# JDAI-CV/CoTNet

Measured on AMD Instinct MI355X. Metric: images/sec CoTNet-50 224^2 fwd+bwd, higher is better.
Workload: dtype bf16; 1 GPU; cotnet50 224x224 fwd+bwd+SGD-nesterov, random init, 1000 classes, NCHW synthetic ImageNet-shaped input resident in HBM; per_gpu_batch=80, global_batch=80, parallelism=dp1, layout=nchw, precision=bf16 weights+activations, fp32 master weights / norm params, fused flat SGD, conv1x1=hip, conv3x3=hip, group_norm9=hip, cot_layer_single_node_enabled=True, grad_sync=none (1 GPU)

## Files before the change

### cotnet_amd/csrc/stem7x7.hip

```cpp
#include "cot_common.h"
#include "mfma_common.h"
#include "cot_host.h"

namespace cot {

constexpr int kStemK = 147, kStemKp = 160, kStemCo = 64;

__device__ __forceinline__ void stem_tap(int k, int& ci, int& kh, int& kw) {
    ci = k / 49;
    const int r = k - 49 * ci;
    kh = r / 7;
    kw = r - 7 * kh;
}

__global__ void __launch_bounds__(256)
stem7x7_fwd_mfma(const bf16_t* __restrict__ x, const bf16_t* __restrict__ w, bf16_t* __restrict__ y, int H, int W, int Ho,
                 int Wo, int tiles_per_image, int64_t total_waves) {
    extern __shared__ __attribute__((aligned(16))) char cot_smem[];
    bf16_t* As = reinterpret_cast<bf16_t*>(cot_smem);
    for (int i = threadIdx.x; i < kStemCo * kStemKp; i += blockDim.x) {
        const int m = i / kStemKp, k = i - m * kStemKp;
        As[i] = k < kStemK ? w[m * kStemK + k] : (bf16_t)0.0f;
    }
    __syncthreads();
    const int64_t wid = (int64_t)blockIdx.x * 4 + (threadIdx.x >> 6);
    if (wid >= total_waves) return;
    const int lane = threadIdx.x & 63, j = lane & 15, g = lane >> 4;
    const int n = uniform((int)(wid / tiles_per_image)), tile = uniform((int)(wid % tiles_per_image));
    const int HWo = Ho * Wo;
    const int p0 = tile * 64 + 4 * j;
    const int oh = min(p0, HWo - 1) / Wo, ow0 = min(p0, HWo - 1) % Wo;
    const int ih0 = 2 * oh - 3, iw0 = 2 * ow0 - 3;
    const bf16_t* xn = x + (int64_t)n * 3 * H * W;

    f32x4_t acc[4][4];
#pragma unroll
    for (int a = 0; a < 4; ++a)
#pragma unroll
        for (int c = 0; c < 4; ++c) acc[a][c] = f32x4_t{0.f, 0.f, 0.f, 0.f};

#pragma unroll
    for (int step = 0; step < kStemKp / 32; ++step) {
        const int kb = 32 * step + 8 * g;
        bf16x8_t bfrag[4];
#pragma unroll
        for (int e = 0; e < 8; ++e) {
            const int k = kb + e;
            int ci, kh, kw;
            stem_tap(min(k, kStemK - 1), ci, kh, kw);
            const int ih = ih0 + kh;
            const bool rok = k < kStemK && ih >= 0 && ih < H && p0 < HWo;
            const bf16_t* row = xn + ((int64_t)ci * H + (rok ? ih : 0)) * W;
#pragma unroll
            for (int cs = 0; cs < 4; ++cs) {
                const int iw = iw0 + 2 * cs + kw;
                bfrag[cs][e] = (rok && iw >= 0 && iw < W) ? row[iw] : (bf16_t)0.0f;
            }
        }
#pragma unroll
        for (int a = 0; a < 4; ++a) {
            bf16x8_t af;
            __builtin_memcpy(&af, __builtin_assume_aligned(As + (16 * a + j) * kStemKp + kb, 16), 16);
#pragma unroll
            for (int cs = 0; cs < 4; ++cs) acc[a][cs] = COT_MFMA_16X16X32_BF16(af, bfrag[cs], acc[a][cs]);
        }
    }
    if (p0 >= HWo) return;
#pragma unroll
    for (int a = 0; a < 4; ++a)
#pragma unroll
        for (int i = 0; i < 4; ++i) {
            const int co = 16 * a + 4 * g + i;
            bf16_t o[4];
#pragma unroll
            for (int cs = 0; cs < 4; ++cs) o[cs] = (bf16_t)acc[a][cs][i];
            store_piece<4, 8>(y + ((int64_t)n * kStemCo + co) * HWo + p0, o, HWo - p0);
        }
}

__global__ void __launch_bounds__(256)
stem7x7_fwd_lds(const bf16_t* __restrict__ x, const bf16_t* __restrict__ w, bf16_t* __restrict__ y, int H, int W, int Ho, int Wo,
                int tiles_per_image, int NR, int RS) {
    constexpr int WS = 168;
    extern __shared__ __attribute__((aligned(16))) char cot_smem[];
    bf16_t* As = reinterpret_cast<bf16_t*>(cot_smem);
    uint16_t* toff = reinterpret_cast<uint16_t*>(As + kStemCo * WS);
    bf16_t* patch = reinterpret_cast<bf16_t*>(toff + kStemKp);
    const int tid = threadIdx.x, lane = tid & 63, wave = tid >> 6, j = lane & 15, g = lane >> 4;
    const int n = blockIdx.x / tiles_per_image, tile = blockIdx.x - n * tiles_per_image;
    const int HWo = Ho * Wo;
    const int pfirst = tile * 256;
    const int ih_base = 2 * (pfirst / Wo) - 3;
    for (int i = tid; i < kStemCo * WS; i += 256) {
        const int m = i / WS, k = i - m * WS;
        As[i] = k < kStemK ? w[m * kStemK + k] : (bf16_t)0.0f;
    }
    if (tid < kStemKp) {
        int ci, kh, kw;
        stem_tap(min(tid, kStemK - 1), ci, kh, kw);
        toff[tid] = (uint16_t)((ci * NR + kh) * RS + kw);
    }
    {
        const int cpr = RS / 8, chunks = 3 * NR * cpr;
        const bf16_t* xn = x + (int64_t)n * 3 * H * W;
        for (int q = tid; q < chunks; q += 256) {
            const int row = q / cpr, c = q - row * cpr;
            const int ci = row / NR, ih = ih_base + (row - ci * NR);
            Vec<bf16_t, 8> v;
#pragma unroll
            for (int e = 0; e < 8; ++e) v.v[e] = (bf16_t)0.0f;
            if (c >= 1 && 8 * (c - 1) < W && ih >= 0 && ih < H) v = ldv<bf16_t, 8>(xn + ((int64_t)ci * H + ih) * W + 8 * (c - 1));
            stv<bf16_t, 8>(patch + (int64_t)row * RS + 8 * c, v);
        }
    }
    __syncthreads();
    const int p0 = pfirst + wave * 64 + 4 * j;
    const int pc = min(p0, HWo - 4);
    const int oh = pc / Wo, ow0 = pc - oh * Wo;
    const uint16_t* pl = reinterpret_cast<const uint16_t*>(patch) + (2 * oh - 3 - ih_base) * RS + 8 + 2 * ow0 - 3;

    f32x4_t acc[4][4];
#pragma unroll
    for (int a = 0; a < 4; ++a)
#pragma unroll
        for (int c = 0; c < 4; ++c) acc[a][c] = f32x4_t{0.f, 0.f, 0.f, 0.f};
#pragma unroll
    for (int step = 0; step < kStemKp / 32; ++step) {
        const int kb = 32 * step + 8 * g;
        uint16_t to[8];
        __builtin_memcpy(to, __builtin_assume_aligned(toff + kb, 16), 16);
        uint16_t q[4][8];
#pragma unroll
        for (int e = 0; e < 8; ++e) {
            const uint16_t* pe = pl + to[e];
            const bool kok = step < 4 || kb + e < kStemK;
#pragma unroll
            for (int cs = 0; cs < 4; ++cs) {
                const uint16_t v = pe[2 * cs];
                q[cs][e] = kok ? v : (uint16_t)0;
            }
        }
        bf16x8_t bfrag[4];
#pragma unroll
        for (int cs = 0; cs < 4; ++cs) __builtin_memcpy(&bfrag[cs], q[cs], 16);
#pragma unroll
        for (int a = 0; a < 4; ++a) {
            bf16x8_t af;
            __builtin_memcpy(&af, __builtin_assume_aligned(As + (16 * a + j) * WS + kb, 16), 16);
#pragma unroll
            for (int cs = 0; cs < 4; ++cs) acc[a][cs] = COT_MFMA_16X16X32_BF16(af, bfrag[cs], acc[a][cs]);
        }
    }
    if (p0 >= HWo) return;
#pragma unroll
    for (int a = 0; a < 4; ++a)
#pragma unroll
        for (int i = 0; i < 4; ++i) {
            const int co = 16 * a + 4 * g + i;
            bf16_t o[4];
#pragma unroll
            for (int cs = 0; cs < 4; ++cs) o[cs] = (bf16_t)acc[a][cs][i];
            store_piece<4, 8>(y + ((int64_t)n * kStemCo + co) * HWo + p0, o, HWo - p0);
        }
}

__global__ void __launch_bounds__(256)
stem7x7_wgrad_mfma(const bf16_t* __restrict__ gy, const bf16_t* __restrict__ x, float* __restrict__ part, int N, int H,
                   int W, int Ho, int Wo, int S, int spi, int64_t total_waves) {
    const int64_t wid = (int64_t)blockIdx.x * 4 + (threadIdx.x >> 6);
    if (wid >= total_waves) return;
    const int lane = threadIdx.x & 63, i16 = lane & 15, lg = lane >> 4;
    const int cb = uniform((int)(wid & 1)), s = uniform((int)(wid >> 1));
    const int HWo = Ho * Wo;
    const int T = N * spi, t0 = (int)((int64_t)T * s / S), t1 = (int)((int64_t)T * (s + 1) / S);
    int tci[5], tkh[5], tkw[5];
    bool tok[5];
#pragma unroll
    for (int q = 0; q < 5; ++q) {
        const int k = cb * 80 + q * 16 + i16;
        tok[q] = k < kStemK;
        stem_tap(min(k, kStemK - 1), tci[q], tkh[q], tkw[q]);
    }
    f32x4_t acc[4][5];
#pragma unroll
    for (int a = 0; a < 4; ++a)
#pragma unroll
        for (int q = 0; q < 5; ++q) acc[a][q] = f32x4_t{0.f, 0.f, 0.f, 0.f};

    for (int t = t0; t < t1; ++t) {
        const int n = t / spi, st = t - n * spi;
        const int p = st * 32 + 8 * lg;
        const int oh = p / Wo, ow = p - oh * Wo;
        bf16x8_t af[4], bfr[5];
#pragma unroll
        for (int a = 0; a < 4; ++a)
            __builtin_memcpy(&af[a], __builtin_assume_aligned(gy + ((int64_t)n * kStemCo + 16 * a + i16) * HWo + p, 16), 16);
#pragma unroll
        for (int q = 0; q < 5; ++q) {
            const int ih = 2 * oh - 3 + tkh[q];
            const bool rok = tok[q] && ih >= 0 && ih < H;
            const bf16_t* row = x + (((int64_t)n * 3 + tci[q]) * H + (rok ? ih : 0)) * W;
            const int iw0 = 2 * ow - 3 + tkw[q];
#pragma unroll
            for (int e = 0; e < 8; ++e) {
                const int iw = iw0 + 2 * e;
                bfr[q][e] = (rok && iw >= 0 && iw < W) ? row[iw] : (bf16_t)0.0f;
            }
        }
#pragma unroll
        for (int a = 0; a < 4; ++a)
#pragma unroll
            for (int q = 0; q < 5; ++q) acc[a][q] = COT_MFMA_16X16X32_BF16(af[a], bfr[q], acc[a][q]);
    }
    float* ps = part + (int64_t)s * kStemCo * kStemK;
#pragma unroll
    for (int a = 0; a < 4; ++a)
#pragma unroll
        for (int i = 0; i < 4; ++i) {
            const int co = 16 * a + 4 * lg + i;
#pragma unroll
            for (int q = 0; q < 5; ++q) {
                const int k = cb * 80 + q * 16 + i16;
                if (k < kStemK) ps[co * kStemK + k] = acc[a][q][i];
            }
        }
}

__global__ void __launch_bounds__(256)
stem7x7_wgrad_lds(const bf16_t* __restrict__ gy, const bf16_t* __restrict__ x, float* __restrict__ part, int N, int H, int W, int Ho,
                  int Wo, int S, int RS) {
    extern __shared__ __attribute__((aligned(16))) char cot_smem[];
    bf16_t* const patch = reinterpret_cast<bf16_t*>(cot_smem);
    const int tid = threadIdx.x, lane = tid & 63, wave = tid >> 6, i16 = lane & 15, lg = lane >> 4;
    const int cb = wave & 1, mh = wave >> 1, s = blockIdx.x;
    const int HWo = Ho * Wo, ppi = Ho / 2;
    const int T = N * ppi, t0 = (int)((int64_t)T * s / S), t1 = (int)((int64_t)T * (s + 1) / S);
    const int cpr = RS / 8, chunks = 27 * cpr;
    constexpr int NCH = 4;
    int toff[5];
    bool tok[5];
#pragma unroll
    for (int q = 0; q < 5; ++q) {
        const int k = cb * 80 + q * 16 + i16;
        int ci, kh, kw;
        stem_tap(min(k, kStemK - 1), ci, kh, kw);
        tok[q] = k < kStemK;
        toff[q] = (ci * 9 + kh) * RS + 8 - 3 + kw;
    }
    f32x4_t acc[2][5];
#pragma unroll
    for (int a = 0; a < 2; ++a)
#pragma unroll
        for (int q = 0; q < 5; ++q) acc[a][q] = f32x4_t{0.f, 0.f, 0.f, 0.f};
    Vec<bf16_t, 8> hold[NCH];
    auto fetch = [&](int t) __attribute__((always_inline)) {
        const int n = t / ppi, pr = t - n * ppi, ih0 = 4 * pr - 3;
        const bf16_t* xn = x + (int64_t)n * 3 * H * W;
#pragma unroll
        for (int j = 0; j < NCH; ++j) {
            const int qd = j * 256 + tid;
#pragma unroll
            for (int e = 0; e < 8; ++e) hold[j].v[e] = (bf16_t)0.0f;
            if (qd < chunks) {
                const int row = qd / cpr, c = qd - row * cpr;
                const int ci = row / 9, ih = ih0 + (row - ci * 9);
                if (c >= 1 && 8 * (c - 1) < W && ih >= 0 && ih < H) hold[j] = ldv<bf16_t, 8>(xn + ((int64_t)ci * H + ih) * W + 8 * (c - 1));
            }
        }
    };
    auto put = [&](int buf) __attribute__((always_inline)) {
#pragma unroll
        for (int j = 0; j < NCH; ++j) {
            const int qd = j * 256 + tid;
            if (qd < chunks) stv<bf16_t, 8>(patch + (int64_t)buf * 27 * RS + (int64_t)qd * 8, hold[j]);
        }
    };
    if (t0 < t1) {
        fetch(t0);
        put(0);
    }
    __syncthreads();
    for (int t = t0; t < t1; ++t) {
        const int buf = (t - t0) & 1;
        if (t + 1 < t1) fetch(t + 1);
        const int n = t / ppi, pr = t - n * ppi;
        const uint16_t* pb = reinterpret_cast<const uint16_t*>(patch) + buf * 27 * RS;
        const bf16_t* gyn = gy + (int64_t)n * kStemCo * HWo + (int64_t)(2 * pr) * Wo;
        for (int ks = 0; ks < 2 * Wo; ks += 32) {
            const int p = ks + 8 * lg;
            const int r2 = p >= Wo ? 1 : 0, ow = p - r2 * Wo;
            const int pbase = 2 * r2 * RS + 2 * ow;
            bf16x8_t af[2], bfr[5];
#pragma unroll
            for (int a = 0; a < 2; ++a)
                __builtin_memcpy(&af[a], __builtin_assume_aligned(gyn + (int64_t)(32 * mh + 16 * a + i16) * HWo + p, 16), 16);
#pragma unroll
            for (int q = 0; q < 5; ++q) {
                const uint16_t* pe = pb + pbase + toff[q];
                uint16_t v[8];
#pragma unroll
                for (int e = 0; e < 8; ++e) v[e] = tok[q] ? pe[2 * e] : (uint16_t)0;
                __builtin_memcpy(&bfr[q], v, 16);
            }
#pragma unroll
            for (int a = 0; a < 2; ++a)
#pragma unroll
                for (int q = 0; q < 5; ++q) acc[a][q] = COT_MFMA_16X16X32_BF16(af[a], bfr[q], acc[a][q]);
        }
        if (t + 1 < t1) put(buf ^ 1);
        __syncthreads();
    }
    float* ps = part + (int64_t)s * kStemCo * kStemK;
#pragma unroll
    for (int a = 0; a < 2; ++a)
#pragma unroll
        for (int i = 0; i < 4; ++i) {
            const int co = 32 * mh + 16 * a + 4 * lg + i;
#pragma unroll
            for (int q = 0; q < 5; ++q) {
                const int k = cb * 80 + q * 16 + i16;
                if (k < kStemK) ps[co * kStemK + k] = acc[a][q][i];
            }
        }
}

static bool stem_geometry(int H, int W, int* Ho, int* Wo) {
    *Ho = (H + 6 - 7) / 2 + 1;
    *Wo = (W + 6 - 7) / 2 + 1;
    return H > 0 && W > 0 && (*Wo % 8) == 0 && ((*Ho * *Wo) % 32) == 0;
}

int g_stem_lds = 1;
static int stem_wgrad_lds_slices(int N, int H, int W, int Ho, int Wo) {
    if (!g_stem_lds || W % 8 != 0 || (2 * Wo) % 32 != 0 || (Ho & 1) || 27 * ((W + 16) / 8) > 4 * 256) return 0;
    const int64_t T = (int64_t)N * (Ho / 2);
    int64_t S = T / 8;
    if (S > 1024) S = 1024;
    return (int)(S < 1 ? 1 : S);
}
int stem7x7_splits(int N, int H, int W) {
    int Ho, Wo;
    if (!stem_geometry(H, W, &Ho, &Wo)) return 0;
    if (const int sl = stem_wgrad_lds_slices(N, H, W, Ho, Wo)) return sl;
    const int64_t T = (int64_t)N * (Ho * Wo / 32);
    int64_t S = 512;
    if (S > T / 16) S = T / 16;
    return (int)(S < 1 ? 1 : S);
}

int stem7x7_forward(const void* x, const void* w, void* y, int N, int H, int W, hipStream_t stream) {
    int Ho, Wo;
    if (!stem_geometry(H, W, &Ho, &Wo)) return COT_ERR_UNSUPPORTED;
    if (g_stem_lds && W % 8 == 0 && Wo % 4 == 0 && (Ho * Wo) % 4 == 0) {
        const int rows = 255 / Wo + 2, NR = 2 * (rows - 1) + 7, RS = W + 16;
        const size_t lds = ((size_t)kStemCo * 168 + kStemKp + (size_t)3 * NR * RS) * 2;
        if (lds <= 64 * 1024 && (3 * NR + 6) * RS + 8 < 65536) {
            const int tiles = ceil_div(Ho * Wo, 256);
            COT_LAUNCH(stem7x7_fwd_lds, dim3((unsigned)((int64_t)N * tiles)), dim3(256), lds, stream, (const bf16_t*)x, (const bf16_t*)w,
                       (bf16_t*)y, H, W, Ho, Wo, tiles, NR, RS);
            return check_launch("stem7x7_fwd_lds");
        }
    }
    const int tpi = ceil_div(Ho * Wo, 64);
    const int64_t waves = (int64_t)N * tpi;
    COT_LAUNCH(stem7x7_fwd_mfma, dim3((unsigned)ceil_div64(waves, 4)), dim3(256), kStemCo * kStemKp * 2, stream,
               (const bf16_t*)x, (const bf16_t*)w, (bf16_t*)y, H, W, Ho, Wo, tpi, waves);
    return check_launch("stem7x7_fwd_mfma");
}

int stem7x7_wgrad(const void* gy, const void* x, void* gw, float* workspace, int N, int H, int W, hipStream_t stream) {
    int Ho, Wo;
    if (!stem_geometry(H, W, &Ho, &Wo)) return COT_ERR_UNSUPPORTED;
    if (const int SL = stem_wgrad_lds_slices(N, H, W, Ho, Wo)) {
        const int RS = W + 16;
        COT_LAUNCH(stem7x7_wgrad_lds, dim3((unsigned)SL), dim3(256), (size_t)2 * 27 * RS * 2, stream, (const bf16_t*)gy, (const bf16_t*)x,
                   workspace, N, H, W, Ho, Wo, SL, RS);
        int rc = check_launch("stem7x7_wgrad_lds");
        if (rc) return rc;
        return conv1x1_wgrad_reduce_launch(workspace, SL, kStemCo, kStemK, 0, gw, nullptr, stream);
    }
    const int S = stem7x7_splits(N, H, W), spi = Ho * Wo / 32;
    const int64_t waves = (int64_t)S * 2;
    COT_LAUNCH(stem7x7_wgrad_mfma, dim3((unsigned)ceil_div64(waves, 4)), dim3(256), 0, stream, (const bf16_t*)gy,
               (const bf16_t*)x, workspace, N, H, W, Ho, Wo, S, spi, waves);
    int rc = check_launch("stem7x7_wgrad_mfma");
    if (rc) return rc;
    return conv1x1_wgrad_reduce_launch(workspace, S, kStemCo, kStemK, 0, gw, nullptr, stream);
}

}
```

Before: 5961 images/s.

## Restructure 7x7 stem conv around kernel-row K packing with persistent, prefetched tiles

Reorders the stem reduction dimension by kernel row: each 8-wide K chunk holds one (channel, kh) row of 7 taps plus a zero pad, so B fragments come from contiguous vector reads instead of per-element gathers. The weights are pre-swizzled into per-lane MFMA fragment order in LDS. The forward LDS kernel becomes persistent, processing 8 tiles per workgroup and prefetching the next tile's input patch into registers while the current tile computes. Weight-gradient patches are split into even/odd column planes and run through a ring-buffered gy load loop, and the slice cap drops from 1024 to 512. K grows from 160 to 192 slots, so more MFMA work is padding, and the forward kernel may request more than 64KB of LDS, which can lower occupancy.

```diff
diff --git a/cotnet_amd/csrc/stem7x7.hip b/cotnet_amd/csrc/stem7x7.hip
--- a/cotnet_amd/csrc/stem7x7.hip
+++ b/cotnet_amd/csrc/stem7x7.hip
@@ -1,10 +1,15 @@
 #include "cot_common.h"
 #include "mfma_common.h"
+#include "conv_lds_common.h"
 #include "cot_host.h"
 
 namespace cot {
 
 constexpr int kStemK = 147, kStemKp = 160, kStemCo = 64;
+constexpr int kStemRows = 21, kStemSteps = 6;
+constexpr int kStemWFrag = 4 * kStemSteps * 64;
+constexpr int kStemTilesPerWg = 8;
+constexpr int kStemWgradSlices = 512;
 
 __device__ __forceinline__ void stem_tap(int k, int& ci, int& kh, int& kw) {
     ci = k / 49;
@@ -13,15 +18,28 @@
     kw = r - 7 * kh;
 }
 
+__device__ __forceinline__ void stem_stage_weights(const bf16_t* __restrict__ w, bf16_t* Af, int tid) {
+    for (int f = tid; f < kStemWFrag; f += 256) {
+        const int q = f >> 6, lane = f & 63, a = q / kStemSteps, s = q - a * kStemSteps;
+        const int co = 16 * a + (lane & 15), r = 4 * s + (lane >> 4);
+        Vec<bf16_t, 8> v;
+#pragma unroll
+        for (int e = 0; e < 8; ++e) v.v[e] = (bf16_t)0.0f;
+        if (r < kStemRows) {
+            const Vec<bf16_t, 7> t = ldv<bf16_t, 7>(w + co * kStemK + 7 * r);
+#pragma unroll
+            for (int e = 0; e < 7; ++e) v.v[e] = t.v[e];
+        }
+        stv<bf16_t, 8>(Af + 8 * f, v);
+    }
+}
+
 __global__ void __launch_bounds__(256)
 stem7x7_fwd_mfma(const bf16_t* __restrict__ x, const bf16_t* __restrict__ w, bf16_t* __restrict__ y, int H, int W, int Ho,
                  int Wo, int tiles_per_image, int64_t total_waves) {
     extern __shared__ __attribute__((aligned(16))) char cot_smem[];
-    bf16_t* As = reinterpret_cast<bf16_t*>(cot_smem);
-    for (int i = threadIdx.x; i < kStemCo * kStemKp; i += blockDim.x) {
-        const int m = i / kStemKp, k = i - m * kStemKp;
-        As[i] = k < kStemK ? w[m * kStemK + k] : (bf16_t)0.0f;
-    }
+    bf16_t* Af = reinterpret_cast<bf16_t*>(cot_smem);
+    stem_stage_weights(w, Af, threadIdx.x);
     __syncthreads();
     const int64_t wid = (int64_t)blockIdx.x * 4 + (threadIdx.x >> 6);
     if (wid >= total_waves) return;
@@ -40,27 +58,25 @@
         for (int c = 0; c < 4; ++c) acc[a][c] = f32x4_t{0.f, 0.f, 0.f, 0.f};
 
 #pragma unroll
-    for (int step = 0; step < kStemKp / 32; ++step) {
-        const int kb = 32 * step + 8 * g;
+    for (int step = 0; step < kStemSteps; ++step) {
+        const int r = 4 * step + g, rc = min(r, kStemRows - 1);
+        const int ci = (rc >= 7) + (rc >= 14), ih = ih0 + rc - 7 * ci;
+        const bool rok = r < kStemRows && ih >= 0 && ih < H && p0 < HWo;
+        const bf16_t* row = xn + ((int64_t)ci * H + (rok ? ih : 0)) * W;
         bf16x8_t bfrag[4];
 #pragma unroll
-        for (int e = 0; e < 8; ++e) {
-            const int k = kb + e;
-            int ci, kh, kw;
-            stem_tap(min(k, kStemK - 1), ci, kh, kw);
-            const int ih = ih0 + kh;
-            const bool rok = k < kStemK && ih >= 0 && ih < H && p0 < HWo;
-            const bf16_t* row = xn + ((int64_t)ci * H + (rok ? ih : 0)) * W;
-#pragma unroll
-            for (int cs = 0; cs < 4; ++cs) {
-                const int iw = iw0 + 2 * cs + kw;
+        for (int cs = 0; cs < 4; ++cs) {
+#pragma unroll
+            for (int e = 0; e < 7; ++e) {
+                const int iw = iw0 + 2 * cs + e;
                 bfrag[cs][e] = (rok && iw >= 0 && iw < W) ? row[iw] : (bf16_t)0.0f;
             }
+            bfrag[cs][7] = (bf16_t)0.0f;
         }
 #pragma unroll
         for (int a = 0; a < 4; ++a) {
             bf16x8_t af;
-            __builtin_memcpy(&af, __builtin_assume_aligned(As + (16 * a + j) * kStemKp + kb, 16), 16);
+            __builtin_memcpy(&af, __builtin_assume_aligned(Af + 8 * ((a * kStemSteps + step) * 64 + lane), 16), 16);
 #pragma unroll
             for (int cs = 0; cs < 4; ++cs) acc[a][cs] = COT_MFMA_16X16X32_BF16(af, bfrag[cs], acc[a][cs]);
         }
@@ -78,90 +94,134 @@
         }
 }
 
+constexpr int kStemHold = 5;
+constexpr int kStemRing = 4;
 __global__ void __launch_bounds__(256)
 stem7x7_fwd_lds(const bf16_t* __restrict__ x, const bf16_t* __restrict__ w, bf16_t* __restrict__ y, int H, int W, int Ho, int Wo,
-                int tiles_per_image, int NR, int RS) {
-    constexpr int WS = 168;
+                int tiles_per_image, int NR, int RS, int64_t total_tiles, int tpw) {
     extern __shared__ __attribute__((aligned(16))) char cot_smem[];
-    bf16_t* As = reinterpret_cast<bf16_t*>(cot_smem);
-    uint16_t* toff = reinterpret_cast<uint16_t*>(As + kStemCo * WS);
-    bf16_t* patch = reinterpret_cast<bf16_t*>(toff + kStemKp);
+    bf16_t* Af = reinterpret_cast<bf16_t*>(cot_smem);
+    bf16_t* patch = Af + 8 * kStemWFrag;
     const int tid = threadIdx.x, lane = tid & 63, wave = tid >> 6, j = lane & 15, g = lane >> 4;
-    const int n = blockIdx.x / tiles_per_image, tile = blockIdx.x - n * tiles_per_image;
     const int HWo = Ho * Wo;
-    const int pfirst = tile * 256;
-    const int ih_base = 2 * (pfirst / Wo) - 3;
-    for (int i = tid; i < kStemCo * WS; i += 256) {
-        const int m = i / WS, k = i - m * WS;
-        As[i] = k < kStemK ? w[m * kStemK + k] : (bf16_t)0.0f;
-    }
-    if (tid < kStemKp) {
-        int ci, kh, kw;
-        stem_tap(min(tid, kStemK - 1), ci, kh, kw);
-        toff[tid] = (uint16_t)((ci * NR + kh) * RS + kw);
-    }
-    {
-        const int cpr = RS / 8, chunks = 3 * NR * cpr;
+    stem_stage_weights(w, Af, tid);
+    int roff[kStemSteps];
+#pragma unroll
+    for (int s = 0; s < kStemSteps; ++s) {
+        const int r = min(4 * s + g, kStemRows - 1), ci = (r >= 7) + (r >= 14);
+        roff[s] = ((ci * NR + r - 7 * ci) * RS) >> 1;
+    }
+    const int cpr = RS / 8, chunks = 3 * NR * cpr, drow = 256 / cpr, dcol = 256 - drow * cpr;
+    const int row_first = tid / cpr, col_first = tid - row_first * cpr;
+    auto next_piece = [&](int& row, int& c) __attribute__((always_inline)) {
+        row += drow;
+        c += dcol;
+        if (c >= cpr) {
+            c -= cpr;
+            ++row;
+        }
+    };
+    auto load_piece = [&](uint32_t (&v)[5], const bf16_t* xn, int ih_base, int row, int c) __attribute__((always_inline)) {
+        const int ci = (row >= NR) + (row >= 2 * NR), ih = ih_base + (row - ci * NR);
+#pragma unroll
+        for (int e = 0; e < 5; ++e) v[e] = 0u;
+        if (ih >= 0 && ih < H) {
+            const bf16_t* xr = xn + ((int64_t)ci * H + ih) * W + 8 * c;
+            if (c >= 2 && 8 * (c - 2) < W) __builtin_memcpy(&v[0], __builtin_assume_aligned(xr - 12, 8), 8);
+            if (c >= 1 && 8 * (c - 1) < W) __builtin_memcpy(&v[2], __builtin_assume_aligned(xr - 8, 16), 12);
+        }
+    };
+    auto make_piece = [&](uint32_t (&o)[4], const uint32_t (&v)[5]) __attribute__((always_inline)) {
+#pragma unroll
+        for (int e = 0; e < 4; ++e) o[e] = (v[e] >> 16) | (v[e + 1] << 16);
+    };
+    uint32_t hold[kStemHold][5];
+    auto fetch = [&](int64_t t) __attribute__((always_inline)) {
+        const int n = (int)(t / tiles_per_image), tile = (int)(t - (int64_t)n * tiles_per_image);
+        const int ih_base = 2 * (tile * 256 / Wo) - 3;
         const bf16_t* xn = x + (int64_t)n * 3 * H * W;
-        for (int q = tid; q < chunks; q += 256) {
-            const int row = q / cpr, c = q - row * cpr;
-            const int ci = row / NR, ih = ih_base + (row - ci * NR);
-            Vec<bf16_t, 8> v;
-#pragma unroll
-            for (int e = 0; e < 8; ++e) v.v[e] = (bf16_t)0.0f;
-            if (c >= 1 && 8 * (c - 1) < W && ih >= 0 && ih < H) v = ldv<bf16_t, 8>(xn + ((int64_t)ci * H + ih) * W + 8 * (c - 1));
-            stv<bf16_t, 8>(patch + (int64_t)row * RS + 8 * c, v);
-        }
-    }
-    __syncthreads();
-    const int p0 = pfirst + wave * 64 + 4 * j;
-    const int pc = min(p0, HWo - 4);
-    const int oh = pc / Wo, ow0 = pc - oh * Wo;
-    const uint16_t* pl = reinterpret_cast<const uint16_t*>(patch) + (2 * oh - 3 - ih_base) * RS + 8 + 2 * ow0 - 3;
-
-    f32x4_t acc[4][4];
-#pragma unroll
-    for (int a = 0; a < 4; ++a)
-#pragma unroll
-        for (int c = 0; c < 4; ++c) acc[a][c] = f32x4_t{0.f, 0.f, 0.f, 0.f};
-#pragma unroll
-    for (int step = 0; step < kStemKp / 32; ++step) {
-        const int kb = 32 * step + 8 * g;
-        uint16_t to[8];
-        __builtin_memcpy(to, __builtin_assume_aligned(toff + kb, 16), 16);
-        uint16_t q[4][8];
-#pragma unroll
-        for (int e = 0; e < 8; ++e) {
-            const uint16_t* pe = pl + to[e];
-            const bool kok = step < 4 || kb + e < kStemK;
+        int row = row_first, c = col_first;
+#pragma unroll
+        for (int i = 0; i < kStemHold; ++i) {
+            if (tid + 256 * i < chunks) load_piece(hold[i], xn, ih_base, row, c);
+            next_piece(row, c);
+        }
+    };
+    const int64_t t0 = (int64_t)blockIdx.x * tpw, t1 = t0 + tpw < total_tiles ? t0 + tpw : total_tiles;
+    if (t0 < t1) fetch(t0);
+    for (int64_t t = t0; t < t1; ++t) {
+        const int n = (int)(t / tiles_per_image), tile = (int)(t - (int64_t)n * tiles_per_image);
+        const int pfirst = tile * 256;
+        const int ih_base = 2 * (pfirst / Wo) - 3;
+        __syncthreads();
+        {
+            int row = row_first, c = col_first;
+#pragma unroll
+            for (int i = 0; i < kStemHold; ++i) {
+                if (tid + 256 * i < chunks) {
+                    uint32_t o[4];
+                    make_piece(o, hold[i]);
+                    __builtin_memcpy(__builtin_assume_aligned(patch + row * RS + 8 * c, 16), o, 16);
+                }
+                next_piece(row, c);
+            }
+            const bf16_t* xn = x + (int64_t)n * 3 * H * W;
+            for (int q = tid + 256 * kStemHold; q < chunks; q += 256) {
+                uint32_t v[5], o[4];
+                load_piece(v, xn, ih_base, row, c);
+                make_piece(o, v);
+                __builtin_memcpy(__builtin_assume_aligned(patch + row * RS + 8 * c, 16), o, 16);
+                next_piece(row, c);
+            }
+        }
+        __syncthreads();
+        if (t + 1 < t1) fetch(t + 1);
+        const int p0 = pfirst + wave * 64 + 4 * j;
+        const int pc = min(p0, HWo - 4);
+        const int oh = pc / Wo, ow0 = pc - oh * Wo;
+        const uint32_t* pl = reinterpret_cast<const uint32_t*>(patch) + (((2 * oh - 3 - ih_base) * RS + 2 * ow0 + 8) >> 1);
+
+        f32x4_t acc[4][4];
+#pragma unroll
+        for (int a = 0; a < 4; ++a)
+#pragma unroll
+            for (int c = 0; c < 4; ++c) acc[a][c] = f32x4_t{0.f, 0.f, 0.f, 0.f};
+#pragma unroll
+        for (int step = 0; step < kStemSteps; ++step) {
+            uint32_t d[8];
+            __builtin_memcpy(d, __builtin_assume_aligned(pl + roff[step], 16), 32);
+            if (4 * step + 3 >= kStemRows) {
+                const bool rok = 4 * step + g < kStemRows;
+#pragma unroll
+                for (int i = 0; i < 8; ++i) d[i] = rok ? d[i] : 0u;
+            }
+            bf16x8_t bfrag[4];
 #pragma unroll
             for (int cs = 0; cs < 4; ++cs) {
-                const uint16_t v = pe[2 * cs];
-                q[cs][e] = kok ? v : (uint16_t)0;
-            }
-        }
-        bf16x8_t bfrag[4];
-#pragma unroll
-        for (int cs = 0; cs < 4; ++cs) __builtin_memcpy(&bfrag[cs], q[cs], 16);
-#pragma unroll
-        for (int a = 0; a < 4; ++a) {
-            bf16x8_t af;
-            __builtin_memcpy(&af, __builtin_assume_aligned(As + (16 * a + j) * WS + kb, 16), 16);
-#pragma unroll
-            for (int cs = 0; cs < 4; ++cs) acc[a][cs] = COT_MFMA_16X16X32_BF16(af, bfrag[cs], acc[a][cs]);
-        }
-    }
-    if (p0 >= HWo) return;
-#pragma unroll
-    for (int a = 0; a < 4; ++a)
-#pragma unroll
-        for (int i = 0; i < 4; ++i) {
-            const int co = 16 * a + 4 * g + i;
-            bf16_t o[4];
-#pragma unroll
-            for (int cs = 0; cs < 4; ++cs) o[cs] = (bf16_t)acc[a][cs][i];
-            store_piece<4, 8>(y + ((int64_t)n * kStemCo + co) * HWo + p0, o, HWo - p0);
-        }
+                const uint32_t q[4] = {d[cs], d[cs + 1], d[cs + 2], d[cs + 3] & 0x0000ffffu};
+                bfrag[cs] = packed_as_frag(q);
+            }
+#pragma unroll
+            for (int a = 0; a < 4; ++a) {
+                bf16x8_t af;
+                __builtin_memcpy(&af, __builtin_assume_aligned(Af + 8 * ((a * kStemSteps + step) * 64 + lane), 16), 16);
+#pragma unroll
+                for (int cs = 0; cs < 4; ++cs) acc[a][cs] = COT_MFMA_16X16X32_BF16(af, bfrag[cs], acc[a][cs]);
+            }
+        }
+        if (p0 < HWo) {
+#pragma unroll
+            for (int a = 0; a < 4; ++a)
+#pragma unroll
+                for (int i = 0; i < 4; ++i) {
+                    const int co = 16 * a + 4 * g + i;
+                    bf16_t o[4];
+#pragma unroll
+                    for (int cs = 0; cs < 4; ++cs) o[cs] = (bf16_t)acc[a][cs][i];
+                    store_piece<4, 8>(y + ((int64_t)n * kStemCo + co) * HWo + p0, o, HWo - p0);
+                }
+        }
+    }
 }
 
 __global__ void __launch_bounds__(256)
@@ -235,24 +295,17 @@
     const int cb = wave & 1, mh = wave >> 1, s = blockIdx.x;
     const int HWo = Ho * Wo, ppi = Ho / 2;
     const int T = N * ppi, t0 = (int)((int64_t)T * s / S), t1 = (int)((int64_t)T * (s + 1) / S);
-    const int cpr = RS / 8, chunks = 27 * cpr;
+    const int RSh = RS / 2, cpr = (W + 16) / 8, chunks = 27 * cpr;
     constexpr int NCH = 4;
-    int toff[5];
-    bool tok[5];
-#pragma unroll
-    for (int q = 0; q < 5; ++q) {
-        const int k = cb * 80 + q * 16 + i16;
-        int ci, kh, kw;
-        stem_tap(min(k, kStemK - 1), ci, kh, kw);
-        tok[q] = k < kStemK;
-        toff[q] = (ci * 9 + kh) * RS + 8 - 3 + kw;
-    }
-    f32x4_t acc[2][5];
+    const int r = 16 * cb + i16;
+    const int rc = min(r, kStemRows - 1), rci = (rc >= 7) + (rc >= 14);
+    const int roff = ((rci * 9 + rc - 7 * rci) * RS) >> 1;
+    f32x4_t acc[2][7];
 #pragma unroll
     for (int a = 0; a < 2; ++a)
 #pragma unroll
-        for (int q = 0; q < 5; ++q) acc[a][q] = f32x4_t{0.f, 0.f, 0.f, 0.f};
-    Vec<bf16_t, 8> hold[NCH];
+        for (int q = 0; q < 7; ++q) acc[a][q] = f32x4_t{0.f, 0.f, 0.f, 0.f};
+    uint32_t hold[NCH][4];
     auto fetch = [&](int t) __attribute__((always_inline)) {
         const int n = t / ppi, pr = t - n * ppi, ih0 = 4 * pr - 3;
         const bf16_t* xn = x + (int64_t)n * 3 * H * W;
@@ -260,11 +313,12 @@
         for (int j = 0; j < NCH; ++j) {
             const int qd = j * 256 + tid;
 #pragma unroll
-            for (int e = 0; e < 8; ++e) hold[j].v[e] = (bf16_t)0.0f;
+            for (int e = 0; e < 4; ++e) hold[j][e] = 0u;
             if (qd < chunks) {
                 const int row = qd / cpr, c = qd - row * cpr;
                 const int ci = row / 9, ih = ih0 + (row - ci * 9);
-                if (c >= 1 && 8 * (c - 1) < W && ih >= 0 && ih < H) hold[j] = ldv<bf16_t, 8>(xn + ((int64_t)ci * H + ih) * W + 8 * (c - 1));
+                if (c >= 1 && 8 * (c - 1) < W && ih >= 0 && ih < H)
+                    __builtin_memcpy(hold[j], __builtin_assume_aligned(xn + ((int64_t)ci * H + ih) * W + 8 * (c - 1), 16), 16);
             }
         }
     };
@@ -272,7 +326,15 @@
 #pragma unroll
         for (int j = 0; j < NCH; ++j) {
             const int qd = j * 256 + tid;
-            if (qd < chunks) stv<bf16_t, 8>(patch + (int64_t)buf * 27 * RS + (int64_t)qd * 8, hold[j]);
+            if (qd < chunks) {
+                const int row = qd / cpr, c = qd - row * cpr;
+                const uint32_t* h = hold[j];
+                const uint32_t ev[2] = {(h[0] & 0x0000ffffu) | (h[1] << 16), (h[2] & 0x0000ffffu) | (h[3] << 16)};
+                const uint32_t od[2] = {(h[0] >> 16) | (h[1] & 0xffff0000u), (h[2] >> 16) | (h[3] & 0xffff0000u)};
+                bf16_t* pr = patch + ((int64_t)buf * 27 + row) * RS + 4 * c;
+                __builtin_memcpy(__builtin_assume_aligned(pr, 8), ev, 8);
+                __builtin_memcpy(__builtin_assume_aligned(pr + RSh, 8), od, 8);
+            }
         }
     };
     if (t0 < t1) {
@@ -280,48 +342,65 @@
         put(0);
     }
     __syncthreads();
-    for (int t = t0; t < t1; ++t) {
-        const int buf = (t - t0) & 1;
-        if (t + 1 < t1) fetch(t + 1);
-        const int n = t / ppi, pr = t - n * ppi;
-        const uint16_t* pb = reinterpret_cast<const uint16_t*>(patch) + buf * 27 * RS;
-        const bf16_t* gyn = gy + (int64_t)n * kStemCo * HWo + (int64_t)(2 * pr) * Wo;
-        for (int ks = 0; ks < 2 * Wo; ks += 32) {
-            const int p = ks + 8 * lg;
-            const int r2 = p >= Wo ? 1 : 0, ow = p - r2 * Wo;
-            const int pbase = 2 * r2 * RS + 2 * ow;
-            bf16x8_t af[2], bfr[5];
-#pragma unroll
-            for (int a = 0; a < 2; ++a)
-                __builtin_memcpy(&af[a], __builtin_assume_aligned(gyn + (int64_t)(32 * mh + 16 * a + i16) * HWo + p, 16), 16);
-#pragma unroll
-            for (int q = 0; q < 5; ++q) {
-                const uint16_t* pe = pb + pbase + toff[q];
-                uint16_t v[8];
-#pragma unroll
-                for (int e = 0; e < 8; ++e) v[e] = tok[q] ? pe[2 * e] : (uint16_t)0;
-                __builtin_memcpy(&bfr[q], v, 16);
-            }
-#pragma unroll
-            for (int a = 0; a < 2; ++a)
-#pragma unroll
-                for (int q = 0; q < 5; ++q) acc[a][q] = COT_MFMA_16X16X32_BF16(af[a], bfr[q], acc[a][q]);
-        }
-        if (t + 1 < t1) put(buf ^ 1);
-        __syncthreads();
-    }
+    const int spp = 2 * Wo / 32;
+    bf16x8_t af[kStemRing][2];
+    int l_n = t0 / ppi, l_pr = t0 - l_n * ppi, l_ks = 0;
+    auto load_step = [&](int slot, int) __attribute__((always_inline)) {
+        const bf16_t* g0 = gy + ((int64_t)l_n * kStemCo + 32 * mh + i16) * HWo + (int64_t)(2 * l_pr) * Wo + l_ks + 8 * lg;
+#pragma unroll
+        for (int a = 0; a < 2; ++a) __builtin_memcpy(&af[slot][a], __builtin_assume_aligned(g0 + (int64_t)16 * a * HWo, 16), 16);
+        l_ks += 32;
+        if (l_ks >= 2 * Wo) {
+            l_ks = 0;
+            if (++l_pr == ppi) {
+                l_pr = 0;
+                ++l_n;
+            }
+        }
+    };
+    int m_t = t0, m_ks = 0;
+    auto multiply_slot = [&](int slot) __attribute__((always_inline)) {
+        const int buf = (m_t - t0) & 1;
+        if (m_ks == 0 && m_t + 1 < t1) fetch(m_t + 1);
+        const int p = m_ks + 8 * lg;
+        const int r2 = p >= Wo ? 1 : 0, ow = p - r2 * Wo;
+        const uint32_t* pw = reinterpret_cast<const uint32_t*>(patch) + ((buf * 27 * RS + 2 * r2 * RS + ow) >> 1) + roff;
+        bf16x8_t bfr[7];
+#pragma unroll
+        for (int q = 0; q < 7; ++q) {
+            constexpr int kD[7] = {2, 3, 3, 4, 4, 5, 5};
+            const int D = kD[q];
+            uint32_t d[8];
+            __builtin_memcpy(d, __builtin_assume_aligned(pw + (((q + 1) & 1) * RSh >> 1), 16), 32);
+            uint32_t v[4];
+#pragma unroll
+            for (int i = 0; i < 4; ++i) v[i] = (D & 1) ? (d[D / 2 + i] >> 16) | (d[D / 2 + i + 1] << 16) : d[D / 2 + i];
+            bfr[q] = packed_as_frag(v);
+        }
+#pragma unroll
+        for (int a = 0; a < 2; ++a)
+#pragma unroll
+            for (int q = 0; q < 7; ++q) acc[a][q] = COT_MFMA_16X16X32_BF16(af[slot][a], bfr[q], acc[a][q]);
+        m_ks += 32;
+        if (m_ks >= 2 * Wo) {
+            if (m_t + 1 < t1) put(buf ^ 1);
+            __syncthreads();
+            m_ks = 0;
+            ++m_t;
+        }
+    };
+    ring_loop<kStemRing>((t1 - t0) * spp, load_step, multiply_slot);
     float* ps = part + (int64_t)s * kStemCo * kStemK;
-#pragma unroll
-    for (int a = 0; a < 2; ++a)
-#pragma unroll
-        for (int i = 0; i < 4; ++i) {
-            const int co = 32 * mh + 16 * a + 4 * lg + i;
-#pragma unroll
-            for (int q = 0; q < 5; ++q) {
-                const int k = cb * 80 + q * 16 + i16;
-                if (k < kStemK) ps[co * kStemK + k] = acc[a][q][i];
-            }
-        }
+    if (r < kStemRows) {
+#pragma unroll
+        for (int a = 0; a < 2; ++a)
+#pragma unroll
+            for (int i = 0; i < 4; ++i) {
+                const int co = 32 * mh + 16 * a + 4 * lg + i;
+#pragma unroll
+                for (int q = 0; q < 7; ++q) ps[co * kStemK + 7 * r + q] = acc[a][q][i];
+            }
+    }
 }
 
 static bool stem_geometry(int H, int W, int* Ho, int* Wo) {
@@ -335,7 +414,7 @@
     if (!g_stem_lds || W % 8 != 0 || (2 * Wo) % 32 != 0 || (Ho & 1) || 27 * ((W + 16) / 8) > 4 * 256) return 0;
     const int64_t T = (int64_t)N * (Ho / 2);
     int64_t S = T / 8;
-    if (S > 1024) S = 1024;
+    if (S > kStemWgradSlices) S = kStemWgradSlices;
     return (int)(S < 1 ? 1 : S);
 }
 int stem7x7_splits(int N, int H, int W) {
@@ -353,17 +432,24 @@
     if (!stem_geometry(H, W, &Ho, &Wo)) return COT_ERR_UNSUPPORTED;
     if (g_stem_lds && W % 8 == 0 && Wo % 4 == 0 && (Ho * Wo) % 4 == 0) {
         const int rows = 255 / Wo + 2, NR = 2 * (rows - 1) + 7, RS = W + 16;
-        const size_t lds = ((size_t)kStemCo * 168 + kStemKp + (size_t)3 * NR * RS) * 2;
-        if (lds <= 64 * 1024 && (3 * NR + 6) * RS + 8 < 65536) {
+        const size_t budget = ((size_t)kStemCo * 168 + kStemKp + (size_t)3 * NR * RS) * 2;
+        if (budget <= 64 * 1024 && (3 * NR + 6) * RS + 8 < 65536) {
             const int tiles = ceil_div(Ho * Wo, 256);
-            COT_LAUNCH(stem7x7_fwd_lds, dim3((unsigned)((int64_t)N * tiles)), dim3(256), lds, stream, (const bf16_t*)x, (const bf16_t*)w,
-                       (bf16_t*)y, H, W, Ho, Wo, tiles, NR, RS);
+            const int64_t total = (int64_t)N * tiles;
+            const size_t lds = (size_t)kStemWFrag * 16 + (size_t)3 * NR * RS * 2;
+            static std::atomic<uint32_t> raised{0};
+            if (lds > 64 * 1024 && !raise_dynamic_lds_once(raised, reinterpret_cast<const void*>(&stem7x7_fwd_lds))) {
+                set_error(COT_ERR_LAUNCH, "stem7x7_fwd_lds: %zu bytes of dynamic LDS refused", lds);
+                return COT_ERR_LAUNCH;
+            }
+            COT_LAUNCH(stem7x7_fwd_lds, dim3((unsigned)ceil_div64(total, kStemTilesPerWg)), dim3(256), lds,
+                       stream, (const bf16_t*)x, (const bf16_t*)w, (bf16_t*)y, H, W, Ho, Wo, tiles, NR, RS, total, kStemTilesPerWg);
             return check_launch("stem7x7_fwd_lds");
         }
     }
     const int tpi = ceil_div(Ho * Wo, 64);
     const int64_t waves = (int64_t)N * tpi;
-    COT_LAUNCH(stem7x7_fwd_mfma, dim3((unsigned)ceil_div64(waves, 4)), dim3(256), kStemCo * kStemKp * 2, stream,
+    COT_LAUNCH(stem7x7_fwd_mfma, dim3((unsigned)ceil_div64(waves, 4)), dim3(256), kStemWFrag * 16, stream,
                (const bf16_t*)x, (const bf16_t*)w, (bf16_t*)y, H, W, Ho, Wo, tpi, waves);
     return check_launch("stem7x7_fwd_mfma");
 }
@@ -372,7 +458,7 @@
     int Ho, Wo;
     if (!stem_geometry(H, W, &Ho, &Wo)) return COT_ERR_UNSUPPORTED;
     if (const int SL = stem_wgrad_lds_slices(N, H, W, Ho, Wo)) {
-        const int RS = W + 16;
+        const int RS = 2 * ((W / 2 + 8 + 7) / 8 * 8);
         COT_LAUNCH(stem7x7_wgrad_lds, dim3((unsigned)SL), dim3(256), (size_t)2 * 27 * RS * 2, stream, (const bf16_t*)gy, (const bf16_t*)x,
                    workspace, N, H, W, Ho, Wo, SL, RS);
         int rc = check_launch("stem7x7_wgrad_lds");
```

New measurement: 6008 images/s, median of 6. About the same (+0.8%).
